# ZhangT-tech/MoCA-Video

Measured on AMD Instinct MI355X. Metric: denoising UNet-steps/sec @16x320x512 fp16, higher is better.
Workload: dtype f16

## Files before the change

include/moca_hip.h:

```cpp
#ifndef MOCA_HIP_H
#define MOCA_HIP_H

#include <stdint.h>

#ifdef __cplusplus
extern "C" {
#endif

#define MOCA_OK            0
#define MOCA_E_BADARG     -1
#define MOCA_E_LAUNCH     -2
#define MOCA_E_NODEVICE   -3
#define MOCA_E_GRAPH      -4

#define MOCA_A_LINEAR   0
#define MOCA_A_CONV3X3  1
#define MOCA_A_TCONV3   2

#define MOCA_EP_GEGLU   1
#define MOCA_EP_OUT_F32 2
#define MOCA_FORCE_SMALL_TILE 4
#define MOCA_EP_COLSUM 16
#define MOCA_EP_LN     32
#define MOCA_EP_GELU    8
// ... 203 lines not shown
    float* momentum;
    float* queue;
    float* x_prev;
    float* pred_x0;
    const float* coef;
    const int32_t* win_start;
    const float* mask;
    const float* mask_sums;
    const int32_t* mask_frame;
    const float* enh;
    const float* cond;
    const float* sam_eff;
    const int32_t* sam_idx;
    float cfg_scale, beta, one_minus_beta, gamma, one_minus_gamma;
    int32_t nW, C, Q, f, HW, wb_from;
} moca_fifo_step_params;
int moca_fifo_step_windows_f32(const moca_fifo_step_params* p, void* stream);
int moca_sam_select_masks_f32(const float* cand, const int32_t* cand_off, const int32_t* ncand, const int64_t* t_rows, float* eff,
                              int32_t* eff_idx, int32_t nW, int32_t f, int32_t HW, void* stream);
int moca_fifo_advance_f32(moca_fifo_state* state, float* queue, const float* newframe, float* emitted, int32_t n_slots,
                          int32_t emit_frame, float* mask, float* mask_sums, int32_t C, int32_t Q, int32_t HW, void* stream);
int moca_fifo_prepare_queue_f32(const float* z, const float* noise, float* queue, const float* coef_z, const float* coef_noise,
                                const int32_t* frame_idx, int32_t BC, int32_t Tz, int32_t Q, int32_t HW, void* stream);
int moca_base_set_timestep(const moca_fifo_state* state, const int64_t* table, int32_t S, int64_t* rows, int32_t n, void* stream);
int moca_base_ddim_step_f32(moca_fifo_state* state, float* x, const float* eps_c, const float* eps_u, const float* noise,
                            float* pred_x0, const float* coef, int32_t S, float cfg_scale, int32_t use_scale, int64_t n, void* stream);
#define MOCA_DDPM_X0 1
#define MOCA_DDPM_CLIP 2
#define MOCA_DDPM_SCALE 4
#define MOCA_DDPM_MASK_C0 8
int moca_ddpm_step_f32(moca_fifo_state* state, const float* x, float* out, const float* eps_c, const float* eps_u,
                       const float* noise, float* x_recon, float* mean, const float* mask, const float* x0,
                       const float* noise_q, const float* coef, const int64_t* t, int64_t t_stride, int32_t B, int32_t n_tab,
                       int64_t per, int64_t mask_inner, float cfg_scale, float temperature, int32_t flags, void* stream);
int moca_mask_frame_sums_f32(const float* mask, float* sums, int32_t frames, int32_t HW, void* stream);

int moca_freq_mix_3d_f32(const float* x, const float* noise, const float* lpf, float* out,
                         int32_t C, int32_t T, int32_t H, int32_t W, float* ws, void* stream);
int64_t moca_freq_mix_ws_bytes(int32_t C, int32_t T, int32_t H, int32_t W);
int moca_freq_filter_f32(float* lpf, int32_t T, int32_t H, int32_t W, int32_t type, int32_t n,
                         double d_s, double d_t, void* stream);

int moca_graph_begin(void* stream);
int moca_graph_end(void* stream, void** graph_exec_out);
int moca_graph_launch(void* graph_exec, void* stream);
int moca_graph_destroy(void* graph_exec);
int moca_stream_create(void** stream_out);
// ... 30 lines not shown
```

moca_video_amd/csrc/fifo.hip:

```cpp
#include "common.h"

namespace {

__device__ __forceinline__ void philox_round(uint32_t (&c)[4], uint32_t k0, uint32_t k1) {
    const uint64_t p0 = (uint64_t)0xD2511F53u * c[0];
    const uint64_t p1 = (uint64_t)0xCD9E8D57u * c[2];
    const uint32_t n0 = (uint32_t)(p1 >> 32) ^ c[1] ^ k0;
    const uint32_t n2 = (uint32_t)(p0 >> 32) ^ c[3] ^ k1;
    c[1] = (uint32_t)p1;
    c[3] = (uint32_t)p0;
    c[0] = n0;
    c[2] = n2;
}

__device__ __forceinline__ void philox4x32_10(uint32_t (&c)[4], uint32_t k0, uint32_t k1) {
#pragma unroll
    for (int r = 0; r < 10; ++r) {
        philox_round(c, k0, k1);
        k0 += 0x9E3779B9u;
        k1 += 0xBB67AE85u;
    }
}

__global__ __launch_bounds__(256) void fifo_randn_kernel(const moca_fifo_state* __restrict__ st, float* __restrict__ out, int64_t n) {
// ... 102 lines not shown
__global__ __launch_bounds__(256) void fifo_advance_copy_kernel(const moca_fifo_state* __restrict__ st, float* __restrict__ queue,
                                                                const float* __restrict__ newframe, float* __restrict__ emitted,
                                                                int n_slots, int emit_frame, float* __restrict__ mask,
                                                                float* __restrict__ mask_sums, int C, int Q, int HW) {
    const int head = st->head;
    const int slot = n_slots > 0 ? st->iter % n_slots : 0;
    const int ef = (head + emit_frame) % Q, tail = (head + Q - 1) % Q;
    for (int64_t i = (int64_t)blockIdx.x * 256 + threadIdx.x; i < (int64_t)C * HW; i += (int64_t)gridDim.x * 256) {
        const int p = (int)(i % HW), c = (int)(i / HW);
        if (emitted) emitted[(int64_t)slot * C * HW + i] = queue[((int64_t)c * Q + ef) * HW + p];
        queue[((int64_t)c * Q + head) * HW + p] = newframe[i];
        if (mask && c == 0) mask[(int64_t)head * HW + p] = mask[(int64_t)tail * HW + p];
    }
    if (mask_sums && blockIdx.x == 0 && threadIdx.x == 0) mask_sums[head] = mask_sums[tail];
}

__global__ void fifo_advance_bump_kernel(moca_fifo_state* st, int Q) {
    st->head = (st->head + 1) % Q;
    st->iter = st->iter + 1;
    st->ext_noise = 0;
}

__global__ __launch_bounds__(256) void base_set_timestep_kernel(const moca_fifo_state* __restrict__ st, const int64_t* __restrict__ table,
                                                                int S, int64_t* __restrict__ rows, int n) {
    const int64_t t = table[S - 1 - st->iter % S];
    for (int i = blockIdx.x * 256 + threadIdx.x; i < n; i += gridDim.x * 256) rows[i] = t;
}

__global__ __launch_bounds__(256) void base_step_kernel(const moca_fifo_state* __restrict__ st, float* __restrict__ x,
                                                        const float* __restrict__ eps_c, const float* __restrict__ eps_u,
                                                        const float* __restrict__ noise, float* __restrict__ pred_x0,
                                                        const float* __restrict__ coef, int S, float cfg_scale, int use_scale, int64_t n) {
    const float* cf = coef + (int64_t)(S - 1 - st->iter % S) * 8;
    const float sqrt_at = cf[0], sqrt_aprev = cf[1], sigma_t = cf[2], s1m = cf[3], dir_coef = cf[4], scale_t = cf[5], scale_prev = cf[6];
    for (int64_t i = (int64_t)blockIdx.x * 256 + threadIdx.x; i < n; i += (int64_t)gridDim.x * 256) {
        float et = eps_c[i];
        if (eps_u) {
            const float u = eps_u[i];
            et = u + cfg_scale * (et - u);
        }
        float p0 = (x[i] - s1m * et) / sqrt_at;
        const float dir = dir_coef * et;
        const float nz = sigma_t * noise[i];
        float xp;
        if (use_scale) {
            p0 = p0 / scale_t;
            xp = sqrt_aprev * scale_prev * p0 + dir + nz;
        } else {
            xp = sqrt_aprev * p0 + dir + nz;
// ... 169 lines not shown
                                     int32_t emit_frame, float* mask, float* mask_sums, int32_t C, int32_t Q, int32_t HW,
                                     void* stream) {
    if (!state || !queue || !newframe || C <= 0 || Q <= 0 || HW <= 0 || emit_frame < 0 || emit_frame >= Q) return MOCA_E_BADARG;
    if (emitted && n_slots <= 0) return MOCA_E_BADARG;
    if (mask && !mask_sums) return MOCA_E_BADARG;
    hipStream_t st = moca_stream(stream);
    hipLaunchKernelGGL(fifo_advance_copy_kernel, dim3(grid_for((int64_t)C * HW)), dim3(256), 0, st, state, queue, newframe, emitted,
                       n_slots, emit_frame, mask, mask_sums, C, Q, HW);
    MOCA_CHECK_LAUNCH();
    hipLaunchKernelGGL(fifo_advance_bump_kernel, dim3(1), dim3(1), 0, st, state, Q);
    MOCA_CHECK_LAUNCH();
    return MOCA_OK;
}

extern "C" int moca_fifo_prepare_queue_f32(const float* z, const float* noise, float* queue, const float* coef_z, const float* coef_noise,
                                           const int32_t* frame_idx, int32_t BC, int32_t Tz, int32_t Q, int32_t HW, void* stream) {
    if (!z || !noise || !queue || !coef_z || !coef_noise || !frame_idx || BC <= 0 || Tz <= 0 || Q <= 0 || HW <= 0) return MOCA_E_BADARG;
    hipLaunchKernelGGL(fifo_prepare_kernel, dim3(grid_for((int64_t)BC * Q * HW)), dim3(256), 0, moca_stream(stream), z, noise, queue, coef_z,
                       coef_noise, frame_idx, BC, Tz, Q, HW);
    MOCA_CHECK_LAUNCH();
    return MOCA_OK;
}

extern "C" int moca_base_set_timestep(const moca_fifo_state* state, const int64_t* table, int32_t S, int64_t* rows, int32_t n, void* stream) {
    if (!state || !table || !rows || S <= 0 || n <= 0) return MOCA_E_BADARG;
    hipLaunchKernelGGL(base_set_timestep_kernel, dim3(grid_for(n)), dim3(256), 0, moca_stream(stream), state, table, S, rows, n);
    MOCA_CHECK_LAUNCH();
    return MOCA_OK;
}

extern "C" int moca_base_ddim_step_f32(moca_fifo_state* state, float* x, const float* eps_c, const float* eps_u, const float* noise,
                                       float* pred_x0, const float* coef, int32_t S, float cfg_scale, int32_t use_scale, int64_t n,
                                       void* stream) {
    if (!state || !x || !eps_c || !noise || !coef || S <= 0 || n <= 0) return MOCA_E_BADARG;
    hipStream_t st = moca_stream(stream);
    hipLaunchKernelGGL(base_step_kernel, dim3(grid_for(n)), dim3(256), 0, st, state, x, eps_c, eps_u, noise, pred_x0, coef, S, cfg_scale,
                       use_scale, n);
    MOCA_CHECK_LAUNCH();
    hipLaunchKernelGGL(state_bump_kernel, dim3(1), dim3(1), 0, st, state);
    MOCA_CHECK_LAUNCH();
    return MOCA_OK;
}

extern "C" int moca_mask_frame_sums_f32(const float* mask, float* sums, int32_t frames, int32_t HW, void* stream) {
    if (!mask || !sums || frames <= 0 || HW <= 0) return MOCA_E_BADARG;
    hipLaunchKernelGGL(mask_frame_sums_kernel, dim3(frames), dim3(256), 0, moca_stream(stream), mask, sums, HW);
    MOCA_CHECK_LAUNCH();
    return MOCA_OK;
}
// ... 1 lines not shown
```

moca_video_amd/dist.py:

```python
from __future__ import annotations

import os

import torch
import torch.distributed as dist

BUCKET_BYTES = 1 << 30


def init_from_env(backend=None):
    world = int(os.environ.get("WORLD_SIZE", "1"))
    rank = int(os.environ.get("RANK", "0"))
    local = int(os.environ.get("LOCAL_RANK", "0"))
    if world > 1 and not dist.is_initialized():
        os.environ.setdefault("MASTER_ADDR", "127.0.0.1")
        os.environ.setdefault("MASTER_PORT", "29500")
        if backend is None:
            backend = os.environ.get("MOCA_DIST_BACKEND") or ("nccl" if torch.cuda.is_available() else "gloo")
        if backend == "nccl":
            torch.cuda.set_device(local % max(torch.cuda.device_count(), 1))
        dist.init_process_group(backend=backend, rank=rank, world_size=world)
    return rank, local, world


# ... 7 lines not shown
        return 0
    sent = broadcast_tensors([p for p in module.parameters()] + [b for b in module.buffers()], src, bucket_bytes)
    for m in module.modules():
        if hasattr(m, "_invalidate"):
            m._invalidate()
    return sent


def _walk_operands(v, pws, tensors):
    from .ops import PackedWeight
    if isinstance(v, PackedWeight):
        if not v.derived:
            pws.setdefault(id(v), v)
    elif torch.is_tensor(v):
        tensors.append(v)
    elif isinstance(v, (tuple, list)):
        for u in v:
            _walk_operands(u, pws, tensors)


def packed_operands(packed, plans):
    pws, seen_t = {}, []
    for plan in plans:
        for st in plan.steps:
            for v in list(getattr(st, "args", ())) + list(getattr(st, "keywords", {}).values()):
                _walk_operands(v, pws, seen_t)
    norm_ptrs = {}
    for v in packed.values():
        if isinstance(v, tuple) and all(torch.is_tensor(t) for t in v):
            for t in v:
                norm_ptrs[t.data_ptr()] = t
    out, done = [], set()

    def add(t):
        if t is not None and t.data_ptr() not in done:
            done.add(t.data_ptr())
            out.append(t)
    for pw in pws.values():
        add(pw.w); add(pw.bias); add(pw.wsum)
    for t in seen_t:
        if t.data_ptr() in norm_ptrs:
            add(norm_ptrs[t.data_ptr()])
    return out


@torch.no_grad()
def broadcast_packed(model, plans, src=0, bucket_bytes=BUCKET_BYTES, drop_masters=True):
    tensors = packed_operands(model._packed, plans)
    if not dist.is_initialized() or dist.get_world_size() == 1:
        return 0, tensors
    sig = [(tuple(t.shape), str(t.dtype)) for t in tensors]
    ref = [sig if dist.get_rank() == src else None]
    dist.broadcast_object_list(ref, src=src)
    if ref[0] != sig:
        raise RuntimeError("broadcast_packed: this rank's packed operand list differs from rank %d's (different plans built?)" % src)
    sent = broadcast_tensors(tensors, src, bucket_bytes)
    if dist.get_rank() != src:
        model._packed_only = True
        if drop_masters:
            for p in model.parameters():
                p.data = torch.empty(0, dtype=p.dtype, device=p.device)
    return sent, tensors


@torch.no_grad()
def broadcast_tensors(tensors, src=0, bucket_bytes=BUCKET_BYTES):
    sent = 0
    i = 0
    while i < len(tensors):
        dtype, dev = tensors[i].dtype, tensors[i].device
        group, nbytes = [], 0
        while i < len(tensors) and tensors[i].dtype == dtype and (not group or nbytes + tensors[i].numel() * tensors[i].element_size() <= bucket_bytes):
            group.append(tensors[i])
            nbytes += tensors[i].numel() * tensors[i].element_size()
            i += 1
        flat = torch.empty(sum(t.numel() for t in group), dtype=dtype, device=dev)
        if dist.get_rank() == src:
            off = 0
            for t in group:
# ... 44 lines not shown
```

moca_video_amd/fifo_graph.py:

```python
from __future__ import annotations

import ctypes as C
import functools

import numpy as np
import torch

from . import lib as _l
from . import ops
from .freeinit import get_freq_filter
from .plan import _Plan
from .unet import UNetModel, same_fps


def fifo_windows(args):
    f = args.video_length
    n = 2 * args.num_partitions if args.lookahead_denoising else args.num_partitions
    for rank in reversed(range(n)):
        start = rank * (f // 2) if args.lookahead_denoising else rank * f
        yield start, start + f // 2, start + f


def _ptr(t):
    return None if t is None else t.data_ptr()


class FifoEngine:

    @staticmethod
    def supported(model, cond, latents, davis_data=None, sam_masks_fn=None):
        unet = getattr(getattr(model, "model", None), "diffusion_model", None)
        return (isinstance(unet, UNetModel) and isinstance(cond, dict) and "c_crossattn" in cond
                and (davis_data is None or getattr(model, "first_stage_model", None) is not None)
                and sam_masks_fn is None and latents is not None and latents.is_cuda and latents.shape[0] == 1)

# ... 26 lines not shown
            indices = np.concatenate([np.full((f // 2,), 0), indices])
        coef = np.zeros((nW, f, 6), np.float32)
        enh = np.ones((nW, f), np.float32)
        mframe = np.full((nW, f), -1, np.int32)
        t_rows = np.zeros((nW, f), np.int64)
        for w, (s0, _, e0) in enumerate(wins):
            t_rows[w] = timesteps[s0:e0]
            Fm = 0 if masks is None else max(0, min(e0, masks.shape[2]) - s0)
            coef[w], enh[w], mi = sampler.step_tables(indices[s0:e0], timesteps[s0:e0], H, Fm)
            mframe[w] = np.where(mi >= 0, s0 + mi, -1)
        to_dev = lambda a: torch.from_numpy(np.ascontiguousarray(a)).to(dev)
        self.coef, self.enh, self.mframe = to_dev(coef), to_dev(enh), to_dev(mframe)
        self.win_start = to_dev(np.asarray([s0 for s0, _, _ in wins], np.int32))
        cc = torch.cat(cond["c_crossattn"], 1)
        ctxs = [cc.expand(nW, -1, -1)]
        if guided:
            ctxs.append(torch.cat(uc["c_crossattn"], 1).expand(nW, -1, -1))
        segs = tuple((nW, int(c.shape[1])) for c in ctxs)
        B = self.reps * nW
        fps_c = cond.get("fps", 16)
        shared = guided and same_fps([fps_c, uc.get("fps", fps_c)])
        self.gather_reps = 1 if shared or not guided else 2
        self.plan = plan = _Plan(unet, B, f, H, W, segs, torch.float32, dev, shared_x=shared)

        def fps_rows(fp):
            if isinstance(fp, int):
                return torch.full((nW * f,), fp, dtype=torch.int64, device=dev)
            return torch.as_tensor(fp, device=dev).reshape(-1)[:1].to(torch.int64).expand(nW * f)
        fr = [fps_rows(fps_c)] + ([fps_rows(uc.get("fps", fps_c))] if guided else [])
        with torch.cuda.stream(plan.stream):
            plan.t_rows.copy_(to_dev(t_rows).reshape(-1).repeat(self.reps))
            plan.fps_rows.copy_(torch.cat(fr))
            r = 0
            for c in ctxs:
                n = c.shape[0] * c.shape[1]
                plan.ctx[r:r + n].copy_(c.reshape(n, -1))
                r += n
        f32 = dict(dtype=torch.float32, device=dev)
        self.queue = latents[0].to(torch.float32).reshape(Cc, Q, HW).clone()
        st = _l.FifoState(0, 0, seed & 0xffffffff, (seed >> 32) & 0xffffffff, 0)
        self.state = torch.frombuffer(bytearray(bytes(st)), dtype=torch.int32).to(dev)
        n_win = nW * Cc * f * HW
        self.noise = torch.zeros(n_win + 2 * Cc * HW, **f32)
        self.moments = None
        if anchor_moments is not None:
            self.moments = anchor_moments.to(dev, torch.float32).reshape(2 * Cc, HW).contiguous()
# ... 53 lines not shown
            _l.check(lib.moca_fifo_randn_f32(st_, _l.ptr(self.noise), self.noise.numel(), S()), "moca_fifo_randn_f32")
            early_anchor = self.moments is None and self.lookahead
            _l.check(lib.moca_fifo_gather_windows_f32(st_, q_, _l.ptr(plan.x_in), _l.ptr(self.anchor) if early_anchor else None,
                                                      _l.ptr(self.win_start), nW, self.gather_reps, Cc, Q, f, HW, S()), "moca_fifo_gather_windows_f32")

        def post():
            if self.sam_capacity > 0:
                _l.check(lib.moca_sam_select_masks_f32(_l.ptr(self.sam_cand), _l.ptr(self.sam_tab[0]), _l.ptr(self.sam_tab[1]),
                                                       _l.ptr(plan.t_rows), _l.ptr(self.sam_eff), _l.ptr(self.sam_idx), nW, f, HW, S()),
                         "moca_sam_select_masks_f32")
            _l.check(lib.moca_fifo_step_windows_f32(C.byref(p), S()), "moca_fifo_step_windows_f32")
            if self.moments is None and not self.lookahead:
                _l.check(lib.moca_fifo_gather_windows_f32(st_, q_, None, _l.ptr(self.anchor), None, 0, 1, Cc, Q, f, HW, S()),
                         "moca_fifo_gather_windows_f32")
            if self.moments is not None:
                _l.check(lib.moca_gaussian_sample_f32(_l.ptr(self.moments), _l.ptr(self.noise[n_win + Cc * HW:]), _l.ptr(self.anchor), 1, Cc, HW,
                                                      float(scale_factor), S()), "moca_gaussian_sample_f32")
            _l.check(lib.moca_freq_mix_3d_f32(_l.ptr(self.anchor), _l.ptr(self.noise[n_win:n_win + Cc * HW]), _l.ptr(self.lpf), _l.ptr(self.newframe),
                                              Cc, 1, H, W, _l.ptr(self.mix_ws), S()), "moca_freq_mix_3d_f32")
            _l.check(lib.moca_fifo_advance_f32(st_, q_, _l.ptr(self.newframe), _l.ptr(self.emitted), self.n_slots, self.emit_frame,
                                               _l.ptr(self.mask), _l.ptr(self.mask_sums), Cc, Q, HW, S()), "moca_fifo_advance_f32")
        self.n_unet_launches = len(plan.steps)
        plan.steps = [pre] + plan.steps + [post]
        self.n_iter = 0
        sampler.momentum = self.momentum[nW - 1].view(1, Cc, f, H, W)

    @staticmethod
    def _cond_image(conditioned_image, Cc, HW, dev):
        if conditioned_image is None:
            return torch.zeros(Cc, HW, dtype=torch.float32, device=dev)
        ci = conditioned_image.to(dev)
        if ci.shape[1] != Cc:
            if ci.shape[1] != 3:
                raise ValueError(f"Conditional image must have 3 or 4 channels, got {ci.shape[1]}")
            ci = torch.cat([ci, torch.ones_like(ci[:, :1])], dim=1)
        return ci.to(torch.float32).reshape(-1, Cc, HW)[0].contiguous()

    def _upload_sam(self, sam_masks):
        pool, tab, ev = self._sam_stage[self._sam_turn]
        self._sam_turn ^= 1
        ev.synchronize()
        tab.zero_()
        used, host_runs, dev_copies = 0, [], []
        if sam_masks is not None:
            for w in range(self.nW):
                cw = sam_masks[w]
# ... 11 lines not shown
                    else:
                        pool[used:used + n].copy_(m.to(torch.float32))
                        host_runs.append((used, n))
                    tab[0, w * self.f + i], tab[1, w * self.f + i] = used, n
                    used += n
        for a, n in host_runs:
            self.sam_cand[a:a + n].copy_(pool[a:a + n], non_blocking=True)
        for a, n, m in dev_copies:
            self.sam_cand[a:a + n].copy_(m.to(self.device, torch.float32), non_blocking=True)
        self.sam_tab.copy_(tab, non_blocking=True)
        ev.record(self.plan.stream)

    def set_context(self, cond_ctx):
        c = torch.cat(list(cond_ctx), 1) if isinstance(cond_ctx, (list, tuple)) else cond_ctx
        L = self.plan.segs[0][1]
        if c.dim() != 3 or c.shape[0] != 1 or c.shape[1] != L:
            raise ValueError(f"set_context: the plan's conditional segment holds [1, {L}, D] contexts, got {tuple(c.shape)}")
        plan = self.plan
        cur = torch.cuda.current_stream(self.device)
        src = c.to(self.device)
        plan.stream.wait_stream(cur)
        with torch.cuda.stream(plan.stream):
            plan.set_context([src.expand(self.nW, -1, -1)])
        src.record_stream(plan.stream)

    def step(self, noise=None, shift_noise=None, anchor_noise=None, sam_masks=None):
        plan = self.plan
        cur = torch.cuda.current_stream(self.device)
        plan.stream.wait_stream(cur)
        with torch.cuda.stream(plan.stream):
            if self.sam_capacity > 0:
                self._upload_sam(sam_masks)
            elif sam_masks is not None:
                raise ValueError("this engine was built without sam_capacity")
            if noise is not None:
                n_win = self.nW * self.C * self.f * self.HW
                self.noise[:n_win].view(self.nW, -1).copy_(torch.stack([n.reshape(-1) for n in noise]).to(self.device, torch.float32))
                chw = self.C * self.HW
                self.noise[n_win:n_win + chw].copy_(shift_noise.reshape(-1).to(self.device, torch.float32))
                if anchor_noise is not None:
                    self.noise[n_win + chw:].copy_(anchor_noise.reshape(-1).to(self.device, torch.float32))
                self.state[4:5].fill_(1)
            handle = plan.stream.cuda_stream
            ops.set_stream(handle)
            try:
                plan._launch(handle)
            finally:
                ops.set_stream(None)
        plan.n_runs += 1
        self.n_iter += 1

    def sync_to(self, stream=None):
        (stream or torch.cuda.current_stream(self.device)).wait_stream(self.plan.stream)

    def latents(self):
        self.sync_to()
        head = self.n_iter % self.Q
        return torch.roll(self.queue, -head, dims=1).reshape(1, self.C, self.Q, self.H, self.W)

    def mask_queue(self):
        self.sync_to()
        head = self.n_iter % self.Q
        return None if self.mask is None else torch.roll(self.mask, -head, dims=0).reshape(1, 1, self.Q, self.H, self.W)

    def emitted_frames(self, i0, i1):
# ... 35 lines not shown
        return set(cond.keys()) <= {"c_crossattn", "fps"} and key == "crossattn" and \
            same_fps([cond.get("fps", 16), uc.get("fps", 16)])

    def __init__(self, model, sampler, x, cond, uc, cfg_scale, seed=0, keep_pred_x0=False, features_adapter=None, n_rows=None):
        self.unet = unet = model.model.diffusion_model
        dev = x.device
        self.device = dev
        if unet._packed is None:
            unet._pack()
        B, Cc, T, H, W = x.shape
        self.shape = (B, Cc, T, H, W)
        S = len(sampler.ddim_timesteps) if n_rows is None else int(n_rows)
        if not 1 <= S <= len(sampler.ddim_timesteps):
            raise ValueError(f"n_rows = {n_rows}: the schedule has {len(sampler.ddim_timesteps)} rows")
        self.S = S
        cc, cu = torch.cat(cond["c_crossattn"], 1), torch.cat(uc["c_crossattn"], 1)
        segs = ((B, int(cc.shape[1])), (B, int(cu.shape[1])))
        self.hybrid = getattr(model.model, "conditioning_key", None) != "crossattn"
        concat = cond.get("c_concat") if self.hybrid else None
        pieces = None if concat is None else tuple(int(c.shape[1]) for c in concat)
        unet._check_adapter(features_adapter)
        self.plan = plan = _Plan(unet, 2 * B, T, H, W, segs, torch.float32, dev, shared_x=True, pieces=pieces,
                                 adapter=None if features_adapter is None else unet.adapter_sites)

        def fps_rows(fp):
            if isinstance(fp, int):
                return torch.full((B * T,), fp, dtype=torch.int64, device=dev)
            fp = torch.as_tensor(fp, device=dev).reshape(-1).to(torch.int64)
            return (fp if fp.shape[0] == B else fp[:1].expand(B)).repeat_interleave(T)
        f32 = np.float32
        coef = np.zeros((S, 8), np.float32)
        use_scale = bool(sampler.use_scale)
        for i in range(S):
            a_t, a_prev, sig = f32(sampler.ddim_alphas[i]), f32(sampler.ddim_alphas_prev[i]), f32(sampler.ddim_sigmas[i])
            coef[i, :5] = (np.sqrt(a_t), np.sqrt(a_prev), sig, f32(sampler.ddim_sqrt_one_minus_alphas[i]), np.sqrt(f32(1.) - a_prev - sig * sig))
            coef[i, 5] = f32(sampler.ddim_scale_arr[i]) if use_scale else 1.0
            coef[i, 6] = f32(sampler.ddim_scale_arr_prev[i]) if use_scale else 1.0
        self.coef = torch.from_numpy(coef).to(dev)
        self.t_table = torch.from_numpy(np.ascontiguousarray(np.asarray(sampler.ddim_timesteps, dtype=np.int64)[:S])).to(dev)
        self.enc_coef = tuple(c.to(dev) for c in sampler.encode_tables())
        self.state = torch.zeros(8, dtype=torch.int32, device=dev)
        self.enc_state = torch.zeros(8, dtype=torch.int32, device=dev)
        n = x.numel()
        self.noise = torch.zeros(n, dtype=torch.float32, device=dev)
        self.pred_x0 = torch.empty(n, dtype=torch.float32, device=dev) if keep_pred_x0 else None
        self._fps_rows = fps_rows
        self.reset(x, cond, uc, seed, features_adapter=features_adapter)
        lib = _l.load()
        eps = plan.out.reshape(2 * B, -1)
        st_ = _l.ptr(self.state)
        S_ = lambda: C.c_void_p(ops.current_stream())

        def pre():
            _l.check(lib.moca_base_set_timestep(st_, _l.ptr(self.t_table), S, _l.ptr(plan.t_rows), plan.t_rows.numel(), S_()), "moca_base_set_timestep")
            _l.check(lib.moca_fifo_randn_f32(st_, _l.ptr(self.noise), n, S_()), "moca_fifo_randn_f32")

        def post():
            _l.check(lib.moca_base_ddim_step_f32(st_, _l.ptr(plan.x_in), _l.ptr(eps[:B]), _l.ptr(eps[B:]), _l.ptr(self.noise), _l.ptr(self.pred_x0),
                                                 _l.ptr(self.coef), S, float(cfg_scale), 1 if use_scale else 0, n, S_()), "moca_base_ddim_step_f32")
        plan.steps = [pre] + plan.steps + [post]

    def reset(self, x, cond, uc, seed=0, features_adapter=None):
        plan, dev = self.plan, self.device
        if (features_adapter is None) != (plan.adapter_in is None):
            raise ValueError("features_adapter goes with an engine built for it")
        B = self.shape[0]
        fps_c, fps_u = (16, 16) if self.hybrid else (cond.get("fps", 16), uc.get("fps", 16))
        if not same_fps([fps_c, fps_u]):
            raise ValueError("BaseEngine shares the UNet prefix between the two guidance branches: their fps must be equal")
        cc, cu = (torch.cat(c["c_crossattn"], 1).expand(B, -1, -1) for c in (cond, uc))
        st = _l.FifoState(0, 0, seed & 0xffffffff, (seed >> 32) & 0xffffffff, 0)
        cur = torch.cuda.current_stream(dev)
        plan.stream.wait_stream(cur)
        with torch.cuda.stream(plan.stream):
            self.state.copy_(torch.frombuffer(bytearray(bytes(st)), dtype=torch.int32))
            st.iter = -1
            self.enc_state.copy_(torch.frombuffer(bytearray(bytes(st)), dtype=torch.int32))
            plan.x_in.copy_(x.to(torch.float32))
            plan.fps_rows.copy_(torch.cat([self._fps_rows(fps_c), self._fps_rows(fps_u)]))
            plan.set_context([cc, cu])
            if features_adapter is not None:
                plan.set_adapter(list(features_adapter))
            if plan.pieces is not None:
                ops.set_stream(plan.stream.cuda_stream)
                try:
                    plan.set_concat(cond["c_concat"])
                finally:
                    ops.set_stream(None)
        cur.wait_stream(plan.stream)
        self.n_iter = 0

    def encode(self, x0, t_index, noise=None):
        plan, dev = self.plan, self.device
        B = self.shape[0]
        if tuple(x0.shape) != tuple(self.shape):
            raise ValueError(f"x0 {tuple(x0.shape)} does not match the engine's latents {tuple(self.shape)}")
        t = torch.as_tensor(t_index)
        t = t.reshape(1).expand(B) if t.dim() == 0 else t
        n_tab = int(self.enc_coef[0].shape[0])
        if t.dim() != 1 or t.shape[0] != B:
            raise ValueError(f"t_index must be one schedule index or [{B}] of them, got {tuple(t.shape)}")
        if not t.is_cuda and (int(t.min()) < 0 or int(t.max()) >= n_tab):
            raise IndexError(f"index {t.tolist()} is out of bounds for the {n_tab}-entry schedule table")
        lib = _l.load()
        n = self.noise.numel()
        cur = torch.cuda.current_stream(dev)
        plan.stream.wait_stream(cur)
        with torch.cuda.stream(plan.stream):
            h = C.c_void_p(plan.stream.cuda_stream)
            src = x0.to(dev, torch.float32).contiguous()
            t_d = t.to(dev, torch.int64).contiguous()
            if noise is not None:
                self.noise.copy_(noise.reshape(-1).to(dev, torch.float32))
            else:
                _l.check(lib.moca_fifo_randn_f32(_l.ptr(self.enc_state), _l.ptr(self.noise), n, h), "moca_fifo_randn_f32")
            _l.check(lib.moca_q_sample_f32(_l.ptr(src), _l.ptr(self.noise), _l.ptr(plan.x_in), _l.ptr(self.enc_coef[0]), _l.ptr(self.enc_coef[1]),
                                           _l.ptr(t_d), B, n_tab, n // B, h), "moca_q_sample_f32")
        src.record_stream(plan.stream)
        t_d.record_stream(plan.stream)

    def step(self, noise=None):
        plan = self.plan
        cur = torch.cuda.current_stream(self.device)
        plan.stream.wait_stream(cur)
        with torch.cuda.stream(plan.stream):
            if noise is not None:
                self.noise.copy_(noise.reshape(-1).to(self.device, torch.float32))
                self.state[4:5].fill_(1)
            handle = plan.stream.cuda_stream
            ops.set_stream(handle)
            try:
                plan._launch(handle)
            finally:
                ops.set_stream(None)
        plan.n_runs += 1
        self.n_iter += 1

    def latents(self):
        torch.cuda.current_stream(self.device).wait_stream(self.plan.stream)
        return self.plan.x_in.clone()

    def last_pred_x0(self):
        torch.cuda.current_stream(self.device).wait_stream(self.plan.stream)
        return None if self.pred_x0 is None else self.pred_x0.view(self.shape).clone()

    def close(self):
        self.plan.close()


class DdpmEngine:

# ... 41 lines not shown
        self.state = torch.zeros(8, dtype=torch.int32, device=dev)
        n = x.numel()
        self.n = n
        self.n_pad = (n + 3) // 4 * 4
        self.masked = mask is not None
        self.noise = torch.zeros(self.n_pad + n if self.masked else n, dtype=torch.float32, device=dev)
        self.mask = self.x0 = None
        self.mask_inner = 0
        self.flags = model._ddpm_flags(clip=model.clip_denoised)
        if self.masked:
            m, mflag, self.mask_inner = mask_operand(mask, x.shape, dev)
            self.flags |= mflag
            self.mask = torch.empty_like(m)
            self.x0 = torch.empty(n, dtype=torch.float32, device=dev)
        self.x_recon = torch.empty(n, dtype=torch.float32, device=dev) if keep_x_recon else None
        self.reset(x, cond, uc, seed, mask=mask, x0=x0)
        lib = _l.load()
        eps = plan.out.reshape(plan.B, -1)
        st_ = _l.ptr(self.state)
        S_ = lambda: C.c_void_p(ops.current_stream())
        nq = self.noise[self.n_pad:] if self.masked else None

        def pre():
            _l.check(lib.moca_base_set_timestep(st_, _l.ptr(self.t_table), S, _l.ptr(plan.t_rows), plan.t_rows.numel(), S_()), "moca_base_set_timestep")
            _l.check(lib.moca_fifo_randn_f32(st_, _l.ptr(self.noise), self.noise.numel(), S_()), "moca_fifo_randn_f32")

        def post():
            _l.check(lib.moca_ddpm_step_f32(st_, _l.ptr(plan.x_in), _l.ptr(plan.x_in), _l.ptr(eps[:B]), _l.ptr(eps[B:]) if self.guided else None,
                                            _l.ptr(self.noise), _l.ptr(self.x_recon), None, _l.ptr(self.mask), _l.ptr(self.x0), _l.ptr(nq),
                                            _l.ptr(self.coef), _l.ptr(plan.t_rows), T, B, int(self.coef.shape[0]), n // B, self.mask_inner,
                                            float(cfg_scale), 1.0, self.flags, S_()), "moca_ddpm_step_f32")
        plan.steps = [pre] + plan.steps + [post]

    def reset(self, x, cond, uc=None, seed=0, mask=None, x0=None):
        from .ddpm import mask_operand
        plan, dev = self.plan, self.device
        B, T = self.shape[0], self.shape[2]
        if (uc is not None) != self.guided or (mask is not None) != self.masked:
            raise ValueError("guidance and mask go with an engine built for them")
        if tuple(x.shape) != self.shape:
            raise ValueError(f"x {tuple(x.shape)} does not match the engine's latents {self.shape}")

        def fps_rows(fp):
            if isinstance(fp, int):
                return torch.full((B * T,), fp, dtype=torch.int64, device=dev)
            fp = torch.as_tensor(fp, device=dev).reshape(-1).to(torch.int64)
            return (fp if fp.shape[0] == B else fp[:1].expand(B)).repeat_interleave(T)
# ... 58 lines not shown
```

moca_video_amd/lib.py:

```python
from __future__ import annotations

import ctypes as C
import os

import torch

_HERE = os.path.dirname(os.path.abspath(__file__))
LIB_PATH = os.environ.get("MOCA_HIP_LIB") or os.path.join(_HERE, "libmoca_hip.so")

MOCA_A_LINEAR, MOCA_A_CONV3X3, MOCA_A_TCONV3 = 0, 1, 2
MOCA_EP_GEGLU, MOCA_EP_OUT_F32, MOCA_FORCE_SMALL_TILE, MOCA_EP_GELU, MOCA_EP_COLSUM, MOCA_EP_LN = 1, 2, 4, 8, 16, 32
MOCA_EP_ROWSUM, MOCA_EP_LNFOLD, MOCA_EP_GSTAT, MOCA_EP_TATTN, MOCA_EP_SLABS = 64, 128, 256, 512, 1024
MOCA_TUNE_GEMM_W80, MOCA_TUNE_GEMM_G4, MOCA_TUNE_GEMM_SQ256, MOCA_TUNE_GEMM_WIDE, MOCA_TUNE_GN_SLAB, MOCA_TUNE_GEMM_G4P, MOCA_TUNE_GEMM_MF32, MOCA_TUNE_GEMM_SQP, MOCA_TUNE_SQP_WALK = 0, 1, 2, 3, 4, 5, 6, 7, 8
MOCA_TUNE_SLAB_F16 = 9
MOCA_TUNE_GEMM_WS = 10
MOCA_DDPM_X0, MOCA_DDPM_CLIP, MOCA_DDPM_SCALE, MOCA_DDPM_MASK_C0 = 1, 2, 4, 8
(MOCA_ROUTE_SMALL64, MOCA_ROUTE_SMALL128, MOCA_ROUTE_GLDS128, MOCA_ROUTE_GLDS160, MOCA_ROUTE_G4, MOCA_ROUTE_W80, MOCA_ROUTE_W80W,
 MOCA_ROUTE_SQ256, MOCA_ROUTE_G4P, MOCA_ROUTE_SQP, MOCA_ROUTE_TATTN, MOCA_ROUTE_WS) = range(1, 13)

_ERR = {0: "ok", -1: "bad argument (shape/alignment contract)", -2: "HIP launch/runtime error",
        -3: "no gfx950 device", -4: "graph capture/replay failed"}


class MocaHipError(RuntimeError):
# ... 75 lines not shown
    "moca_temporal_attention_long_f16": (C.c_int, [_vp, _vp, _vp, _vp, _i32, _i32, _i32, _i32, _i32, _i32, _f32, _i32, _vp]),
    "moca_ncthw_to_nhwc_f16": (C.c_int, [_vp, _i32, _vp, _i32, _i32, _i32, _i32, _i32, _vp]),
    "moca_ncthw_scatter_f16": (C.c_int, [_vp, _i32, _vp, _i32, _i32, _i32, _i32, _i32, _i32, _vp]),
    "moca_nchw_add_rows_f16": (C.c_int, [_vp, _vp, _i32, _i32, _i32, _i32, _i32, _i32, _vp]),
    "moca_nhwc_to_ncthw": (C.c_int, [_vp, _i32, _vp, _i32, _i32, _i32, _i32, _i32, _vp]),
    "moca_concat_channels_f16": (C.c_int, [_vp, _vp, _vp, _i64, _i32, _i32, _vp]),
    "moca_repeat_f16": (C.c_int, [_vp, _vp, _i64, _i32, _vp]),
    "moca_timestep_embedding_f16": (C.c_int, [_vp, _vp, _i32, _i32, _f32, _vp]),
    "moca_silu_add_rows_f16": (C.c_int, [_vp, _i32, _vp, _i32, _vp, _i32, _i32, _i32, _vp]),
    "moca_channel_mix_f16": (C.c_int, [_vp, _i32, _vp, _vp, _vp, _i32, _i32, _i32, _i32, _i32, _i32, _f32, _vp]),
    "moca_softmax_rows_f16": (C.c_int, [_vp, _vp, _i64, _i32, _i64, _i64, _f32, _vp]),
    "moca_gaussian_sample_f32": (C.c_int, [_vp, _vp, _vp, _i32, _i32, _i32, _f32, _vp]),
    "moca_cfg_combine_f32": (C.c_int, [_vp, _vp, _vp, _f32, _i64, _vp]),
    "moca_ddim_update_f32": (C.c_int, [_vp, _vp, _vp, _vp, _vp, _f32, _f32, _f32, _f32, _i32, _f32, _f32, _i64, _vp]),
    "moca_q_sample_f32": (C.c_int, [_vp, _vp, _vp, _vp, _vp, _vp, _i32, _i32, _i64, _vp]),
    "moca_fifo_ddim_step_f32": (C.c_int, [_vp, _vp, _vp, _vp, _vp, _vp, _vp, _vp, _vp, _vp, _vp, _vp,
                                          _i32, _i32, _i32, _i32, _i32, _f32, _f32, _f32, _f32, _vp]),
    "moca_fifo_randn_f32": (C.c_int, [_vp, _vp, _i64, _vp]),
    "moca_fifo_gather_windows_f32": (C.c_int, [_vp, _vp, _vp, _vp, _vp, _i32, _i32, _i32, _i32, _i32, _i32, _vp]),
    "moca_fifo_step_windows_f32": (C.c_int, [C.POINTER(FifoStepParams), _vp]),
    "moca_sam_select_masks_f32": (C.c_int, [_vp, _vp, _vp, _vp, _vp, _vp, _i32, _i32, _i32, _vp]),
    "moca_fifo_advance_f32": (C.c_int, [_vp, _vp, _vp, _vp, _i32, _i32, _vp, _vp, _i32, _i32, _i32, _vp]),
    "moca_fifo_prepare_queue_f32": (C.c_int, [_vp, _vp, _vp, _vp, _vp, _vp, _i32, _i32, _i32, _i32, _vp]),
    "moca_base_set_timestep": (C.c_int, [_vp, _vp, _i32, _vp, _i32, _vp]),
    "moca_base_ddim_step_f32": (C.c_int, [_vp, _vp, _vp, _vp, _vp, _vp, _vp, _i32, _f32, _i32, _i64, _vp]),
    "moca_ddpm_step_f32": (C.c_int, [_vp] * 13 + [_i64, _i32, _i32, _i64, _i64, _f32, _f32, _i32, _vp]),
    "moca_mask_frame_sums_f32": (C.c_int, [_vp, _vp, _i32, _i32, _vp]),
    "moca_freq_mix_3d_f32": (C.c_int, [_vp, _vp, _vp, _vp, _i32, _i32, _i32, _i32, _vp, _vp]),
    "moca_freq_mix_ws_bytes": (_i64, [_i32, _i32, _i32, _i32]),
    "moca_freq_filter_f32": (C.c_int, [_vp, _i32, _i32, _i32, _i32, _i32, _f64, _f64, _vp]),
    "moca_graph_begin": (C.c_int, [_vp]),
    "moca_graph_end": (C.c_int, [_vp, C.POINTER(_vp)]),
    "moca_graph_launch": (C.c_int, [_vp, _vp]),
    "moca_graph_destroy": (C.c_int, [_vp]),
    "moca_stream_create": (C.c_int, [C.POINTER(_vp)]),
    "moca_stream_destroy": (C.c_int, [_vp]),
    "moca_stream_sync": (C.c_int, [_vp]),
    "moca_event_create": (C.c_int, [C.POINTER(_vp)]),
    "moca_event_record": (C.c_int, [_vp, _vp]),
    "moca_event_elapsed_ms": (C.c_int, [_vp, _vp, C.POINTER(_f32)]),
    "moca_event_destroy": (C.c_int, [_vp]),
    "moca_set_tuning": (C.c_int, [_i32, _i32]),
    "moca_debug_clock_sampler": (C.c_int, [_vp, _i32, _i32, _vp, _vp]),
    "moca_device_info": (C.c_int, [C.c_char_p, _i32, C.POINTER(_i32)]),
    "moca_version": (C.c_char_p, []),
}

# ... 58 lines not shown
```

moca_video_amd/plan.py:

```python
from __future__ import annotations

import ctypes as C
import functools
import os
import warnings

import torch

from . import lib as _l
from . import ops
from .unet import (IMAGE_CONTEXT_MAX, TEXT_CONTEXT_LEN, _BasicTransformerBlock, _CatMap, _Downsample, _FMap, _Pool, _ResBlock,
                   _SpatialTransformer, _TemporalTransformer, _Upsample)

N_CU = 256


def gemm_splits(M, pw):
    nk = pw.w.shape[1] // 64
    tiles = 0
    if pw.N % 160 == 0 and not pw.geglu and M > 160:
        tiles = ((M + 319) // 320) * (pw.N // 160)
        if tiles < 200:
            tiles = 0
    if tiles == 0:
# ... 9 lines not shown
        if nk <= 24:
            return 1
        if nk <= 100:
            return max(1, min(cap, 4))
    return max(1, min(cap, nk // 8))


PREFETCH_MIN_BYTES = int(float(os.environ.get("MOCA_PREFETCH_MIN_MB", "4")) * (1 << 20))
PREFETCH_HOST_FLOP = float(os.environ.get("MOCA_PREFETCH_HOST_GF", "50")) * 1e9
VIRTUAL_CAT = os.environ.get("MOCA_VCAT", "1") != "0"
SPLITK_GN = os.environ.get("MOCA_SKGN", "1") != "0"
GN_FOLD = os.environ.get("MOCA_GNFOLD", "1") != "0"
SPLITK_GN_ALL = os.environ.get("MOCA_SKGN", "1") == "2"
MAX_FRAMES = 32
GSTAT_MAX_PARTIALS = (1 << 11) - 1


def _check_gstat_range(rows):
    if 2 * -(-rows // 160) > GSTAT_MAX_PARTIALS:
        raise ValueError(f"GroupNorm statistics over {rows} rows (frames x pixels of one group) are outside the range of the fixed-point "
                         f"accumulators: at most {GSTAT_MAX_PARTIALS // 2 * 160} rows, e.g. 32 frames of 5115 latent pixels")


class _LNRef:
    __slots__ = ("x", "part", "nparts")

    def __init__(self, x, part, nparts):
        self.x, self.part, self.nparts = x, part, nparts


class _PlanBase:
    _defer_slabs = False

    def __init__(self, model, device):
        self.model = model
        self.device = device
        self.P = model._packed
        self.pool = _Pool(device)
        self.stream = torch.cuda.Stream(device=device) if torch.device(device).type == "cuda" else None
        self.steps = []
        self._pinned = set()
        self.graph = None
        self.graph_failed = False
        self.n_runs = 0
        self._gstat_buf, self._gstat_used, self._last_gemm_step = None, 0, None
        self._last_slabs = None
        self._held = {}
        self._gstat_full = []
        self.reps = 1
        self._prefetch_at = {}
        self.prefetch_on = getattr(model, "weight_prefetch", True)

    def _note_gemm(self, pw):
        if self._last_gemm_step is not None and not pw.derived and pw.w.numel() * pw.w.element_size() >= PREFETCH_MIN_BYTES:
            self._prefetch_at.setdefault(self._last_gemm_step, []).append(pw.w)
        self._last_gemm_step = len(self.steps)

    def _finish_prefetch(self):
        if self.prefetch_on:
            for j, ws in self._prefetch_at.items():
                prod = self.steps[j]
                kw = dict(prod.keywords)
                if 2.0 * kw["M"] * prod.args[1].N * prod.args[1].K < PREFETCH_HOST_FLOP:
                    continue
                kw["prefetch"] = max(ws, key=lambda w: w.numel())
                self.steps[j] = functools.partial(prod.func, *prod.args, **kw)
        self._prefetch_at = {}

    def close(self):
        if self.graph is not None:
            g, self.graph = self.graph, None
            try:
                torch.cuda.synchronize(self.device)
                _l.load().moca_graph_destroy(g)
# ... 594 lines not shown

    def _embed_mlp(self, sq, rows_t):
        m, P, BT = self.model, self.P, self.BT
        te = self.pool.get(BT, m.model_channels)
        self._emit(ops.timestep_embedding, rows_t, te, n=BT, dim=m.model_channels)
        e1 = self.linear(te, BT, P[id(sq[0])])
        s1 = self.pool.get(BT, e1.shape[1])
        self._emit(ops.silu_add_rows, e1, 1, None, 1, s1, rows=BT, Cn=e1.shape[1], silu=True)
        e2 = self.linear(s1, BT, P[id(sq[2])])
        self._release(te, e1, s1)
        return e2

    def _build(self):
        m, P, B, T, H, W = self.model, self.P, self.B, self.T, self.H, self.W
        BT = self.BT
        emb = self._embed_mlp(m.time_embed, self.t_rows)
        femb = self._embed_mlp(m.fps_embedding, self.fps_rows) if m.fps_cond else None
        self.emb_silu = self.pool.get(BT, emb.shape[1])
        self._emit(ops.silu_add_rows, emb, 1, femb, 1, self.emb_silu, rows=BT, Cn=emb.shape[1], silu=True)
        self._release(emb, femb)
        self._pinned.add(self.emb_silu.data_ptr())
        self.emb_all = self.linear(self.emb_silu, BT, P["emb_all"])
        self._pinned.add(self.emb_all.data_ptr())
        self.kv_all = None
        if "ctx_kv_all" in P:
            self.kv_all = self.linear(self.ctx, self.ctx_rows, P["ctx_kv_all"])
            self._pinned.add(self.kv_all.data_ptr())
        self.kv_ip_all = None
        if self.ctx_img is not None:
            self.kv_ip_all = self.linear(self.ctx_img, self.img_rows, P["ctx_kv_ip_all"])
            self._pinned.add(self.kv_ip_all.data_ptr())

        FT = self.Bx * T
        Cpad = m.in_cpad
        if self.pieces is None:
            x8 = self.pool.get(FT * H * W, Cpad)
            self._emit(ops.ncthw_to_nhwc, self.x_in, x8, B=self.Bx, Cin=m.in_channels, T=T, HW=H * W, Cpad=Cpad)
            h = self.conv(_FMap(x8, FT, H, W, Cpad), P[id(m.input_blocks[0][0])])
            self._release(x8)
        else:
            self.x_rows = torch.zeros(FT * H * W, Cpad, dtype=torch.float16, device=self.device)
            self._emit(ops.ncthw_scatter, self.x_in, self.x_rows, B=self.Bx, k=self.kx, T=T, HW=H * W, Cpad=Cpad, c0=0)
            h = self.conv(_FMap(self.x_rows, FT, H, W, Cpad), P[id(m.input_blocks[0][0])])
        hs = []
        for i, module in enumerate(m.input_blocks):
            if i == 0:
                if m.addition_attention:
                    nh = self.transformer(m.init_attn[0], h, False)
                    self._release(h.buf)
                    self._drop_colsum(h)
                    h = nh
            else:
                h = self.run_seq(module, h)
            if self.adapter_in is not None and (i + 1) % 3 == 0:
# ... 21 lines not shown
            cat = self.pool.get(h.M, h.C + skip.C)
            gst = None
            Cc = h.C + skip.C
            if isinstance(module[0], _ResBlock) and Cc % 32 == 0 and \
                    64 <= (Cc // 8) * max(1, 256 // (Cc // 8)) and Cc // 8 <= 1024:
                gst = (self._gstat_slot(h.F * 64), 1)
                self._emit(ops.concat_channels_gstat, h.buf, skip.buf, cat, gst[0], F=h.F, HW=h.H * h.W, C1=h.C, C2=skip.C,
                           frames_per_stat=1)
            else:
                self._emit(ops.concat_channels, h.buf, skip.buf, cat, rows=h.M, C1=h.C, C2=skip.C)
            self._pinned.discard(skip.buf.data_ptr())
            self._drop_colsum(h)
            self._drop_colsum(skip)
            self._release(h.buf, skip.buf)
            h = self.run_seq(module, _FMap(cat, h.F, h.H, h.W, Cc, gstat=gst))
        g = self.gn(h, P[id(m.out[0])], fps=1, eps=1e-5, silu=True)
        self._release(h.buf)
        self._drop_colsum(h)
        o = self.conv(_FMap(g, h.F, h.H, h.W, h.C), P[id(m.out[2])])
        self._release(g)
        self._emit(ops.nhwc_to_ncthw, o.buf, o.C, self.out, B=B, Cout=m.out_channels, T=T, HW=H * W)
        self._release(o.buf)
        self._finish_prefetch()

    def _adapter_add(self, h, FT):
        self._drop_colsum(h)
        assert h.gstat is None and h.gstat_own is None and not h.cs_used
        h.src, h.cs_rows = None, 0
        src = torch.empty(FT, h.C, h.H, h.W, dtype=torch.float32, device=self.device)
        self.adapter_in.append(src)
        self._emit(ops.nchw_add_rows, h.buf, src, F=h.F, Fsrc=FT, Cn=h.C, HW=h.H * h.W)

    def _virtual_cat(self, module, h, skip):
        if not VIRTUAL_CAT or not isinstance(module[0], _ResBlock) or isinstance(module[0].skip_connection, torch.nn.Identity):
            return None
        Cc, HW = h.C + skip.C, h.H * h.W
        if Cc % 32 or h.C % 64 or skip.C % 64 or Cc // 8 > 1024 or h.F != skip.F:
            return None
        pw = self.P[id(module[0].skip_connection)]
        if self._splits(h.M, pw) != 1 or not ops.gemm_cat_ok(h.buf, pw, M=h.M, lda=h.buf.stride(-2), splits=1, a2=(skip.buf, h.C)):
            return None
        gw = Cc // 32
        slot = self._gstat_slot(h.F * 64)

        def retarget(fm, coff):
            rows = fm.colsum[1] if fm.colsum is not None else fm.cs_rows
# ... 103 lines not shown
```

Measured before the change: 61.19.

## Hoist step-invariant embedding and context KV work out of per-step UNet plan

```diff
diff --git a/include/moca_hip.h b/include/moca_hip.h
--- a/include/moca_hip.h
+++ b/include/moca_hip.h
@@ -249,7 +249,9 @@
                           int32_t emit_frame, float* mask, float* mask_sums, int32_t C, int32_t Q, int32_t HW, void* stream);
 int moca_fifo_prepare_queue_f32(const float* z, const float* noise, float* queue, const float* coef_z, const float* coef_noise,
                                 const int32_t* frame_idx, int32_t BC, int32_t Tz, int32_t Q, int32_t HW, void* stream);
-int moca_base_set_timestep(const moca_fifo_state* state, const int64_t* table, int32_t S, int64_t* rows, int32_t n, void* stream);
+int moca_base_set_timestep(const moca_fifo_state* state, const int64_t* table, int32_t S, int64_t* rows, int32_t n,
+                           const void* emb_table, void* emb_rows, int32_t n_samples, int32_t frames, int32_t cols, int32_t ld,
+                           void* stream);
 int moca_base_ddim_step_f32(moca_fifo_state* state, float* x, const float* eps_c, const float* eps_u, const float* noise,
                             float* pred_x0, const float* coef, int32_t S, float cfg_scale, int32_t use_scale, int64_t n, void* stream);
 #define MOCA_DDPM_X0 1
diff --git a/moca_video_amd/csrc/fifo.hip b/moca_video_amd/csrc/fifo.hip
--- a/moca_video_amd/csrc/fifo.hip
+++ b/moca_video_amd/csrc/fifo.hip
@@ -148,9 +148,19 @@
 }
 
 __global__ __launch_bounds__(256) void base_set_timestep_kernel(const moca_fifo_state* __restrict__ st, const int64_t* __restrict__ table,
-                                                                int S, int64_t* __restrict__ rows, int n) {
-    const int64_t t = table[S - 1 - st->iter % S];
+                                                                int S, int64_t* __restrict__ rows, int n, const uint4* __restrict__ emb_table,
+                                                                uint4* __restrict__ emb_rows, int n_samples, int frames, int chunks, int ld8) {
+    const int idx = S - 1 - st->iter % S;
+    const int64_t t = table[idx];
     for (int i = blockIdx.x * 256 + threadIdx.x; i < n; i += gridDim.x * 256) rows[i] = t;
+    if (!emb_table) return;
+    const uint4* __restrict__ src = emb_table + (int64_t)idx * n_samples * chunks;
+    const int64_t total = (int64_t)n_samples * frames * chunks;
+    for (int64_t q = (int64_t)blockIdx.x * 256 + threadIdx.x; q < total; q += (int64_t)gridDim.x * 256) {
+        const int64_t r = q / chunks;
+        const int c = (int)(q - r * chunks);
+        emb_rows[r * ld8 + c] = src[(r / frames) * chunks + c];
+    }
 }
 
 __global__ __launch_bounds__(256) void base_step_kernel(const moca_fifo_state* __restrict__ st, float* __restrict__ x,
@@ -366,9 +376,19 @@
     return MOCA_OK;
 }
 
-extern "C" int moca_base_set_timestep(const moca_fifo_state* state, const int64_t* table, int32_t S, int64_t* rows, int32_t n, void* stream) {
+extern "C" int moca_base_set_timestep(const moca_fifo_state* state, const int64_t* table, int32_t S, int64_t* rows, int32_t n,
+                                      const void* emb_table, void* emb_rows, int32_t n_samples, int32_t frames, int32_t cols, int32_t ld,
+                                      void* stream) {
     if (!state || !table || !rows || S <= 0 || n <= 0) return MOCA_E_BADARG;
-    hipLaunchKernelGGL(base_set_timestep_kernel, dim3(grid_for(n)), dim3(256), 0, moca_stream(stream), state, table, S, rows, n);
+    int64_t work = n;
+    if (emb_table) {
+        if (!emb_rows || n_samples <= 0 || frames <= 0 || cols <= 0 || cols % 8 || ld % 8 || ld < cols) return MOCA_E_BADARG;
+        if (((uintptr_t)emb_table | (uintptr_t)emb_rows) & 15) return MOCA_E_BADARG;
+        const int64_t chunks = (int64_t)n_samples * frames * (cols / 8);
+        if (chunks > work) work = chunks;
+    }
+    hipLaunchKernelGGL(base_set_timestep_kernel, dim3(grid_for(work)), dim3(256), 0, moca_stream(stream), state, table, S, rows, n,
+                       (const uint4*)emb_table, (uint4*)emb_rows, n_samples, frames, cols / 8, ld / 8);
     MOCA_CHECK_LAUNCH();
     return MOCA_OK;
 }
diff --git a/moca_video_amd/dist.py b/moca_video_amd/dist.py
--- a/moca_video_amd/dist.py
+++ b/moca_video_amd/dist.py
@@ -53,7 +53,7 @@
 def packed_operands(packed, plans):
     pws, seen_t = {}, []
     for plan in plans:
-        for st in plan.steps:
+        for st in list(getattr(plan, "hoisted_steps", ())) + list(plan.steps):
             for v in list(getattr(st, "args", ())) + list(getattr(st, "keywords", {}).values()):
                 _walk_operands(v, pws, seen_t)
     norm_ptrs = {}
@@ -86,6 +86,10 @@
     if ref[0] != sig:
         raise RuntimeError("broadcast_packed: this rank's packed operand list differs from rank %d's (different plans built?)" % src)
     sent = broadcast_tensors(tensors, src, bucket_bytes)
+    for plan in plans:
+        invalidate = getattr(plan, "invalidate_hoisted", None)
+        if invalidate is not None:
+            invalidate()
     if dist.get_rank() != src:
         model._packed_only = True
         if drop_masters:
diff --git a/moca_video_amd/fifo_graph.py b/moca_video_amd/fifo_graph.py
--- a/moca_video_amd/fifo_graph.py
+++ b/moca_video_amd/fifo_graph.py
@@ -2,6 +2,7 @@
 
 import ctypes as C
 import functools
+import os
 
 import numpy as np
 import torch
@@ -11,6 +12,8 @@
 from .freeinit import get_freq_filter
 from .plan import _Plan
 from .unet import UNetModel, same_fps
+
+HOIST_INVARIANTS = os.environ.get("MOCA_HOIST_INVARIANTS", "1") != "0"
 
 
 def fifo_windows(args):
@@ -83,6 +86,8 @@
         shared = guided and same_fps([fps_c, uc.get("fps", fps_c)])
         self.gather_reps = 1 if shared or not guided else 2
         self.plan = plan = _Plan(unet, B, f, H, W, segs, torch.float32, dev, shared_x=shared)
+        if HOIST_INVARIANTS:
+            plan.hoist_invariants()
 
         def fps_rows(fp):
             if isinstance(fp, int):
@@ -182,6 +187,8 @@
                                                _l.ptr(self.mask), _l.ptr(self.mask_sums), Cc, Q, HW, S()), "moca_fifo_advance_f32")
         self.n_unet_launches = len(plan.steps)
         plan.steps = [pre] + plan.steps + [post]
+        if plan.hoisted_steps:
+            self._run_hoisted()
         self.n_iter = 0
         sampler.momentum = self.momentum[nW - 1].view(1, Cc, f, H, W)
 
@@ -239,7 +246,20 @@
         plan.stream.wait_stream(cur)
         with torch.cuda.stream(plan.stream):
             plan.set_context([src.expand(self.nW, -1, -1)])
+            if plan.hoisted_steps:
+                self._run_hoisted(emb=False)
         src.record_stream(plan.stream)
+
+    def _run_hoisted(self, emb=True, kv=True):
+        plan = self.plan
+        ops.set_stream(plan.stream.cuda_stream)
+        try:
+            for s in (plan.hoisted_emb if emb else ()) + (plan.hoisted_kv if kv else ()):
+                s()
+        finally:
+            ops.set_stream(None)
+        if emb and kv:
+            plan.hoisted_dirty = False
 
     def step(self, noise=None, shift_noise=None, anchor_noise=None, sam_masks=None):
         plan = self.plan
@@ -258,6 +278,8 @@
                 if anchor_noise is not None:
                     self.noise[n_win + chw:].copy_(anchor_noise.reshape(-1).to(self.device, torch.float32))
                 self.state[4:5].fill_(1)
+            if plan.hoisted_dirty:
+                self._run_hoisted()
             handle = plan.stream.cuda_stream
             ops.set_stream(handle)
             try:
@@ -339,6 +361,10 @@
         unet._check_adapter(features_adapter)
         self.plan = plan = _Plan(unet, 2 * B, T, H, W, segs, torch.float32, dev, shared_x=True, pieces=pieces,
                                  adapter=None if features_adapter is None else unet.adapter_sites)
+        self.emb_table = None
+        if HOIST_INVARIANTS:
+            plan.hoist_invariants()
+            self.emb_table = torch.empty(S, 2 * B, plan.emb_all.shape[1], dtype=torch.float16, device=dev)
 
         def fps_rows(fp):
             if isinstance(fp, int):
@@ -368,8 +394,11 @@
         st_ = _l.ptr(self.state)
         S_ = lambda: C.c_void_p(ops.current_stream())
 
+        emb_cols, emb_ld = int(plan.emb_all.shape[1]), int(plan.emb_all.stride(0))
+
         def pre():
-            _l.check(lib.moca_base_set_timestep(st_, _l.ptr(self.t_table), S, _l.ptr(plan.t_rows), plan.t_rows.numel(), S_()), "moca_base_set_timestep")
+            _l.check(lib.moca_base_set_timestep(st_, _l.ptr(self.t_table), S, _l.ptr(plan.t_rows), plan.t_rows.numel(),
+                                                _l.ptr(self.emb_table), _l.ptr(plan.emb_all), 2 * B, T, emb_cols, emb_ld, S_()), "moca_base_set_timestep")
             _l.check(lib.moca_fifo_randn_f32(st_, _l.ptr(self.noise), n, S_()), "moca_fifo_randn_f32")
 
         def post():
@@ -404,8 +433,28 @@
                     plan.set_concat(cond["c_concat"])
                 finally:
                     ops.set_stream(None)
+            if plan.hoisted_steps:
+                self._refresh_hoisted()
         cur.wait_stream(plan.stream)
         self.n_iter = 0
+
+    def _refresh_hoisted(self):
+        plan = self.plan
+        B2, T, S = 2 * self.shape[0], self.shape[2], self.S
+        ops.set_stream(plan.stream.cuda_stream)
+        try:
+            for c0 in range(0, S, T):
+                k = min(T, S - c0)
+                idx = (c0 + torch.arange(T, device=self.device)).clamp_(max=S - 1)
+                plan.t_rows.view(B2, T).copy_(self.t_table[idx].expand(B2, T))
+                for s in plan.hoisted_emb:
+                    s()
+                self.emb_table[c0:c0 + k].copy_(plan.emb_all.view(B2, T, -1)[:, :k].transpose(0, 1))
+            for s in plan.hoisted_kv:
+                s()
+        finally:
+            ops.set_stream(None)
+        plan.hoisted_dirty = False
 
     def encode(self, x0, t_index, noise=None):
         plan, dev = self.plan, self.device
@@ -444,6 +493,8 @@
             if noise is not None:
                 self.noise.copy_(noise.reshape(-1).to(self.device, torch.float32))
                 self.state[4:5].fill_(1)
+            if plan.hoisted_dirty:
+                self._refresh_hoisted()
             handle = plan.stream.cuda_stream
             ops.set_stream(handle)
             try:
@@ -531,7 +582,8 @@
         nq = self.noise[self.n_pad:] if self.masked else None
 
         def pre():
-            _l.check(lib.moca_base_set_timestep(st_, _l.ptr(self.t_table), S, _l.ptr(plan.t_rows), plan.t_rows.numel(), S_()), "moca_base_set_timestep")
+            _l.check(lib.moca_base_set_timestep(st_, _l.ptr(self.t_table), S, _l.ptr(plan.t_rows), plan.t_rows.numel(), None, None, 0, 0, 0, 0,
+                                                S_()), "moca_base_set_timestep")
             _l.check(lib.moca_fifo_randn_f32(st_, _l.ptr(self.noise), self.noise.numel(), S_()), "moca_fifo_randn_f32")
 
         def post():
diff --git a/moca_video_amd/lib.py b/moca_video_amd/lib.py
--- a/moca_video_amd/lib.py
+++ b/moca_video_amd/lib.py
@@ -121,7 +121,7 @@
     "moca_sam_select_masks_f32": (C.c_int, [_vp, _vp, _vp, _vp, _vp, _vp, _i32, _i32, _i32, _vp]),
     "moca_fifo_advance_f32": (C.c_int, [_vp, _vp, _vp, _vp, _i32, _i32, _vp, _vp, _i32, _i32, _i32, _vp]),
     "moca_fifo_prepare_queue_f32": (C.c_int, [_vp, _vp, _vp, _vp, _vp, _vp, _i32, _i32, _i32, _i32, _vp]),
-    "moca_base_set_timestep": (C.c_int, [_vp, _vp, _i32, _vp, _i32, _vp]),
+    "moca_base_set_timestep": (C.c_int, [_vp, _vp, _i32, _vp, _i32, _vp, _vp, _i32, _i32, _i32, _i32, _vp]),
     "moca_base_ddim_step_f32": (C.c_int, [_vp, _vp, _vp, _vp, _vp, _vp, _vp, _i32, _f32, _i32, _i64, _vp]),
     "moca_ddpm_step_f32": (C.c_int, [_vp] * 13 + [_i64, _i32, _i32, _i64, _i64, _f32, _f32, _i32, _vp]),
     "moca_mask_frame_sums_f32": (C.c_int, [_vp, _vp, _i32, _i32, _vp]),
diff --git a/moca_video_amd/plan.py b/moca_video_amd/plan.py
--- a/moca_video_amd/plan.py
+++ b/moca_video_amd/plan.py
@@ -55,6 +55,14 @@
                          f"accumulators: at most {GSTAT_MAX_PARTIALS // 2 * 160} rows, e.g. 32 frames of 5115 latent pixels")
 
 
+def _without_prefetch(step):
+    if step.keywords.get("prefetch") is None:
+        return step
+    kw = dict(step.keywords)
+    del kw["prefetch"]
+    return functools.partial(step.func, *step.args, **kw)
+
+
 class _LNRef:
     __slots__ = ("x", "part", "nparts")
 
@@ -83,6 +91,8 @@
         self.reps = 1
         self._prefetch_at = {}
         self.prefetch_on = getattr(model, "weight_prefetch", True)
+        self.hoisted_steps = ()
+        self.hoisted_dirty = False
 
     def _note_gemm(self, pw):
         if self._last_gemm_step is not None and not pw.derived and pw.w.numel() * pw.w.element_size() >= PREFETCH_MIN_BYTES:
@@ -723,6 +733,7 @@
         self._pinned.add(self.emb_silu.data_ptr())
         self.emb_all = self.linear(self.emb_silu, BT, P["emb_all"])
         self._pinned.add(self.emb_all.data_ptr())
+        self.emb_range = (0, len(self.steps))
         self.kv_all = None
         if "ctx_kv_all" in P:
             self.kv_all = self.linear(self.ctx, self.ctx_rows, P["ctx_kv_all"])
@@ -731,6 +742,9 @@
         if self.ctx_img is not None:
             self.kv_ip_all = self.linear(self.ctx_img, self.img_rows, P["ctx_kv_ip_all"])
             self._pinned.add(self.kv_ip_all.data_ptr())
+        self.kv_range = (self.emb_range[1], len(self.steps))
+        assert self._last_slabs is None and not self._held
+        invariant = list(self.steps)
 
         FT = self.Bx * T
         Cpad = m.in_cpad
@@ -798,6 +812,24 @@
         self._emit(ops.nhwc_to_ncthw, o.buf, o.C, self.out, B=B, Cout=m.out_channels, T=T, HW=H * W)
         self._release(o.buf)
         self._finish_prefetch()
+        def same_launch(a, b):
+            ka, kb = a.keywords, _without_prefetch(b).keywords
+            return a.func is b.func and len(a.args) == len(b.args) and all(x is y for x, y in zip(a.args, b.args)) and \
+                ka.keys() == kb.keys() and all(ka[k] is kb[k] for k in ka)
+        assert all(a is b or same_launch(a, b) for a, b in zip(invariant, self.steps)), "a step of the invariant prefix was re-targeted"
+
+    def hoist_invariants(self):
+        assert not self.hoisted_steps and self.n_runs == 0 and self.graph is None
+        (e0, e1), (k0, k1) = self.emb_range, self.kv_range
+        assert e0 == 0 and e1 == k0
+        self.hoisted_emb = tuple(_without_prefetch(s) for s in self.steps[e0:e1])
+        self.hoisted_kv = tuple(_without_prefetch(s) for s in self.steps[k0:k1])
+        self.hoisted_steps = self.hoisted_emb + self.hoisted_kv
+        self.steps = self.steps[k1:]
+        self.hoisted_dirty = True
+
+    def invalidate_hoisted(self):
+        self.hoisted_dirty = bool(self.hoisted_steps)
 
     def _adapter_add(self, h, FT):
         self._drop_colsum(h)
```

Result: no change. 61.44, median of 6 (+0.4%).
